# kellerberrin/KGL_Gene

Hardware: AMD Instinct MI355X
Metric: variants·genomes/sec (allele-freq sweep) (higher is better)
Workload: dtype u32

## Files before the change

### kgl_gene_amd/csrc/kgx_inbreed.hip

```cpp
#include <hip/hip_runtime.h>

#include <algorithm>
#include <cmath>
#include <cstdio>
#include <cstdlib>
#include <cstring>
#include <new>
#include <random>
#include <string>
#include <vector>

#include "kgx_kernels_inbreed.h"
#include "kgx_kernels_hall.h"
#include "kgx_kernels_loglik.h"
#include <hipcub/hipcub.hpp>
#include "kgx_internal.h"
#include "kgx_inbreed_plan.h"
#include "kgx_inbreed_buffers.h"

namespace kgx {
namespace {

int require_runtime(std::shared_ptr<Runtime>& rt) {
  rt = current_runtime();
// ... 30 lines not shown
  sw.no_eval_lut = env_int("KGX_K5_NO_EVAL_LUT", 0) != 0;
  sw.no_table_sweep = env_int("KGX_K5_NO_TABLE_SWEEP", 0) != 0;
  sw.no_swar16 = env_int("KGX_K5_NO_SWAR16", 0) != 0;
  sw.eval_gpl = env_int("KGX_K5_EVAL_GPL", 8);
  if (sw.eval_gpl != 4 && sw.eval_gpl != 8) sw.eval_gpl = 8;
  sw.blocks_per_cu = env_int("KGX_K5_BLOCKS_PER_CU", 8);
  sw.eval_resident = env_int("KGX_K5_EVAL_RESIDENT", 2);
  sw.eval_rounds = env_int("KGX_K5_EVAL_ROUNDS", 8);
  sw.sequential_min = env_int("KGX_K5_SEQUENTIAL_MIN", 1 << 16);
  sw.always_guard = env_int("KGX_K5_ALWAYS_GUARD", 0) != 0;
  sw.xcds = static_cast<uint32_t>(std::max(1, env_int("KGX_K5_XCDS", 1)));
  sw.time_small_calls = env_int("KGX_TIME_SMALL_CALLS", 0) != 0;
  sw.keep_scratch_gb = env_int("KGX_KEEP_SCRATCH_GB", -1);
  sw.no_wave = env_int("KGX_K7_NO_WAVE", 0) != 0;
  sw.wave_loci = std::min(kGenomeWaveLoci, std::max(1, env_int("KGX_K7_WAVE_LOCI", 1024)));
  sw.wave_genomes = std::max(1, env_int("KGX_K7_WAVE_GENOMES", algorithm == KGX_ALGO_HALL_ME ? 1024 : 512));
  sw.search_brent = env_str("KGX_K7_SEARCH") == "brent";
  sw.hall_passes = env_int("KGX_K7_HALL_PASSES", 0) != 0;
  sw.golden = env_int("KGX_K7_GOLDEN", 0) != 0;
  sw.estimate_start = env_int("KGX_K7_ESTIMATE_START", 0);
  sw.ll_passes = env_int("KGX_K7_LL_PASSES", 0) != 0;
  sw.ll_het_terms = env_int("KGX_K7_LL_HET_TERMS", 0) != 0;
  sw.ll_dense_per_1024 = env_int("KGX_K7_LL_DENSE_PER_1024", 0);
  sw.class_sweeps = env_int("KGX_K7_CLASS_SWEEPS", 0) != 0;
  sw.class_bytes = env_int("KGX_K7_CLASS_BYTES", 0) != 0;
  sw.order_one_lane = env_int("KGX_K7_ORDER_ONE_LANE", 0) != 0;
  sw.no_pair = env_int("KGX_K7_NO_PAIR", 0) != 0;
  sw.no_compact = env_int("KGX_K7_NO_COMPACT", 0) != 0;
  sw.compact_min_genomes = env_int("KGX_K7_COMPACT_MIN_GENOMES", 2048);
  sw.compact_min_cells = env_int("KGX_K7_COMPACT_MIN_CELLS", 1 << 26);
  sw.trace = env_int("KGX_K7_TRACE", 0) != 0;
  return sw;
}

struct ClassHits {
  unsigned long long* words = nullptr;
  uint64_t word_blocks = 0;
  bool by_bits = false;
  HallClassRows class_rows{};
};

struct EvalTarget {
  const uint32_t* gt;
  uint64_t dwords_per_row, g0, n;
  const uint32_t* index;
  double* f;
// ... 499 lines not shown
    std::fprintf(stderr, "[kgx] HallME step %d: %llu of %llu genomes moved (%llu back to the value before), largest move %.3e\n", it + 1,
                 (unsigned long long)changed, (unsigned long long)n, (unsigned long long)cycling, worst);
    trace_prev2 = trace_prev;
    trace_prev = trace_now;
  }
}

bool InbreedCall::loglik_by_moments(std::vector<uint32_t>& handed_over) {
  const uint64_t n = shape.n;
  const int objective_method = shape.objective_method;
  const bool loglik_moments = plan.loglik_candidate;
  if (objective_method == 1 && !loglik_moments)
    rc = fail(KGX_ESTATE, "kgx_inbreed_objective: this call would not run on the moments (selection size, amax, phase, memory or a switch)");
  if (!(loglik_moments && objective_method != 2 && rc == KGX_OK && gather_moments(true))) {
    if (objective_method == 1 && rc == KGX_OK)
      rc = fail(KGX_ESTATE, "kgx_inbreed_objective: a frequency without a bin, or no room for the hits' words: the passes would run");
    return false;
  }
  uint32_t* const h_totals = m.totals();
  uint32_t n_used = 0;
  try_hip(hipMemcpyAsync(&n_used, h_totals, sizeof(uint32_t), hipMemcpyDeviceToHost, st), KGX_EHIP, "D2H(used bins)");
  try_hip(hipStreamSynchronize(st), KGX_EHIP, "sync");
  unsigned long long* d_search_stats = sw.trace ? m.d_search_stats : nullptr;
  if (d_search_stats) try_hip(hipMemsetAsync(d_search_stats, 0, 8 * sizeof(unsigned long long), st), KGX_EHIP, "memset(search stats)");
  try_hip(hipEventRecord(dev.search_begin, st), KGX_EHIP, "hipEventRecord");
  hipLaunchKernelGGL(k_loglik_search, dim3(static_cast<uint32_t>(n)), dim3(kBlock), loglik_search_lds(n_used), st, m.bins, m.used(), h_totals, b.d_counts, b.d_sums,
                     m.d_smallest_het, n, plan.words_per_block, loglik_classes, b.d_start, objective_method == 1 ? 1 : 0, b.d_f, m.d_needs_passes, h_totals + 2,
                     b.d_running, d_search_stats);
  try_hip(hipGetLastError(), KGX_EHIP, "loglik search launch");
  try_hip(hipEventRecord(dev.search_end, st), KGX_EHIP, "hipEventRecord");
  search_timed = true;
  uint32_t handed = 0;
  unsigned int evaluations = 0;
  try_hip(hipMemcpyAsync(&handed, h_totals + 2, sizeof(uint32_t), hipMemcpyDeviceToHost, st), KGX_EHIP, "D2H(handed over)");
  try_hip(hipMemcpyAsync(&evaluations, b.d_running, sizeof(unsigned int), hipMemcpyDeviceToHost, st), KGX_EHIP, "D2H(evaluations)");
  try_hip(hipStreamSynchronize(st), KGX_EHIP, "sync");
  if (rc != KGX_OK) return false;
  if (d_search_stats) {
    unsigned long long stats[8] = {0};
    try_hip(hipMemcpy(stats, d_search_stats, sizeof(stats), hipMemcpyDeviceToHost), KGX_EHIP, "D2H(search stats)");
    std::fprintf(stderr, "kgx: Loglikelihood search over %llu genomes (%u bins used): %llu evaluations, %llu with cells in their band -- %llu served by kept cells, "
                         "%llu gathers kept, %llu gathers not kept, %llu dense walks; %llu cells listed, %llu blocks looked at\n",
                 (unsigned long long)n, n_used, stats[0], stats[1], stats[2], stats[3], stats[4], stats[5], stats[6], stats[7]);
  }
  dev.last_evaluations = static_cast<int>(evaluations);
  dev.last_path = KGX_PATH_LOGLIK_MOMENTS;
  if (handed) {
    std::vector<uint32_t> flags(n);
    try_hip(hipMemcpyAsync(flags.data(), m.d_needs_passes, n * sizeof(uint32_t), hipMemcpyDeviceToHost, st), KGX_EHIP, "D2H(needs passes)");
    try_hip(hipMemcpyAsync(b.d_keep, b.d_f, n * sizeof(double), hipMemcpyDeviceToDevice, st), KGX_EHIP, "copy(kept results)");
    try_hip(hipMemsetAsync(b.d_running, 0, sizeof(unsigned int), st), KGX_EHIP, "memset(running)");
    try_hip(hipStreamSynchronize(st), KGX_EHIP, "sync");
    for (uint64_t g = 0; g < n; ++g)
      if (flags[g]) {
        handed_over.push_back(static_cast<uint32_t>(g));
        if (sw.trace) std::fprintf(stderr, "kgx: Loglikelihood: genome %llu handed to the passes (reason %u)\n", (unsigned long long)(shape.g0 + g), flags[g]);
      }
    if (rc == KGX_OK) dev.last_path = KGX_PATH_LOGLIK_MOMENTS_AND_PASSES;
  }
  return true;
}

int InbreedCall::loglik_objective() {
  const uint64_t n = shape.n;
  if (shape.objective_method == 2 && rc == KGX_OK) {
    try_hip(hipMemcpyAsync(b.d_f, b.d_start, n * sizeof(double), hipMemcpyDeviceToDevice, st), KGX_EHIP, "copy(points)");
// ... 699 lines not shown
```

### kgl_gene_amd/csrc/kgx_inbreed_buffers.h

```cpp
#ifndef KGX_INBREED_BUFFERS_H
#define KGX_INBREED_BUFFERS_H

#include <type_traits>

#include "kgx_inbreed_plan.h"
#include "kgx_internal.h"
#include "kgx_kernels_loglik.h"

namespace kgx {

template <typename Fn>
void with_bool(bool value, Fn&& fn) {
  if (value) fn(std::true_type{}); else fn(std::false_type{});
}
template <int... Values, typename Fn>
void with_int(int value, Fn&& fn) {
  (void)((value == Values ? (fn(std::integral_constant<int, Values>{}), true) : false) || ...);
}

struct Carver {
  char* base = nullptr;
  ScratchPlan plan;
  template <typename T>
  T* take(size_t bytes) {
// ... 59 lines not shown
constexpr size_t kHallClassWords = 4 * (kHallBins + 1);

struct MomentsBuffers {
  uint32_t classes = 0;
  uint64_t items_per_class = 0;
  size_t padded_records = 0;
  size_t keys_bytes = 0, records_bytes = 0, sort_bytes = 0, sort_stride = 0;
  char* keys = nullptr;
  char* records = nullptr;
  HallRecord* padded = nullptr;
  uint32_t* words = nullptr;
  size_t word_count = 0;
  HallItem* items = nullptr;
  uint32_t* item_blocks = nullptr;
  double* ys = nullptr;
  int8_t* digits = nullptr;
  uint32_t* rows = nullptr;
  uint32_t* slot_of_locus = nullptr;
  char* sort = nullptr;
  double* moments = nullptr;
  double* bins = nullptr;
  uint32_t* d_needs_passes = nullptr;
  unsigned long long *d_smallest_het = nullptr, *d_search_stats = nullptr;

  uint32_t* class_words(uint32_t k) const { return words + k * kHallClassWords; }
  uint32_t* bin_used() const { return words + classes * kHallClassWords; }
  uint32_t* used() const { return bin_used() + (kHallBins + 1); }
  uint32_t* counters() const { return used() + (kHallBins + 1); }
  uint32_t* totals() const { return counters() + classes * 4; }
  HallRecord* padded_of(uint32_t k) const { return padded + static_cast<uint64_t>(k) * padded_records; }
  double* ys_of(uint32_t k) const { return ys ? ys + static_cast<uint64_t>(k) * padded_records : nullptr; }
  HallItem* items_of(uint32_t k) const { return items + static_cast<uint64_t>(k) * items_per_class; }
  uint32_t* item_blocks_of(uint32_t k) const { return item_blocks + static_cast<uint64_t>(k) * (items_per_class + 1); }
  int8_t* digits_of(uint32_t k) const { return digits + static_cast<uint64_t>(k) * padded_records * 32; }
  uint32_t* rows_of(uint32_t k) const { return rows + static_cast<uint64_t>(k) * padded_records; }
};

inline MomentsBuffers carve_moments(Carver& c, const InbreedShape& s, const InbreedPlan& p, size_t sort_bytes) {
  const uint64_t n = s.n, n_sel = s.n_sel;
  const bool planned = p.by_moments(), loglik = p.loglik_candidate;
  MomentsBuffers m;
  m.classes = planned ? p.hall_classes : 0;
  m.items_per_class = p.hall_items;
  m.padded_records = static_cast<size_t>(p.hall_blocks + 1) * kHallBlockLoci;
  m.keys_bytes = (4 * n_sel * sizeof(uint32_t) + 255) / 256 * 256;
  m.records_bytes = (n_sel * sizeof(HallRecord) + 255) / 256 * 256;
  m.keys = c.take<char>(planned ? 2 * m.keys_bytes : 0);
  m.records = c.take<char>(planned ? 2 * m.records_bytes : 0);
  m.padded = c.take<HallRecord>(m.classes * m.padded_records * sizeof(HallRecord));
  m.word_count = m.classes * kHallClassWords + 2 * (kHallBins + 1) + (m.classes + 1) * 4;
  m.words = c.take<uint32_t>(planned ? m.word_count * sizeof(uint32_t) : 0);
  m.items = c.take<HallItem>(m.classes * m.items_per_class * sizeof(HallItem));
  m.item_blocks = c.take<uint32_t>(m.classes * (m.items_per_class + 1) * sizeof(uint32_t));
  m.ys = c.take<double>(loglik ? m.classes * m.padded_records * sizeof(double) : 0);
  if (!loglik) m.ys = nullptr;
  m.digits = c.take<int8_t>(p.hall_mfma ? m.classes * m.padded_records * 32 : 0);
  m.rows = c.take<uint32_t>(p.hall_mfma ? m.classes * m.padded_records * sizeof(uint32_t) : 0);
  m.slot_of_locus = c.take<uint32_t>(p.hall_bits_planned ? m.classes * p.sel_pitch * sizeof(uint32_t) : 0);
  if (!p.hall_bits_planned) m.slot_of_locus = nullptr;
  m.sort_bytes = sort_bytes;
  m.sort_stride = (sort_bytes + 255) / 256 * 256;
  m.sort = c.take<char>(2 * m.sort_stride);
  m.moments = c.take<double>(m.items_per_class * kHallMoments * n * sizeof(double));
  m.bins = c.take<double>(planned ? static_cast<size_t>(kHallBins) * kHallMoments * n * sizeof(double) : 0);
  m.d_needs_passes = c.take<uint32_t>(loglik ? n * sizeof(uint32_t) : 0);
  m.d_smallest_het = c.take<unsigned long long>(sizeof(unsigned long long));
  m.d_search_stats = c.take<unsigned long long>(8 * sizeof(unsigned long long));
  return m;
}

}

#endif
```

### kgl_gene_amd/csrc/kgx_inbreed_plan.h

```cpp
#ifndef KGX_INBREED_PLAN_H
#define KGX_INBREED_PLAN_H

#include <cassert>
#include <cstddef>
#include <stdint.h>

#include "kgx_inbreed_constants.h"

namespace kgx {

constexpr int kAlgoRitlandLocus = 0, kAlgoSimple = 1, kAlgoHallME = 2, kAlgoLoglikelihood = 3;

struct InbreedSwitches {
  bool generic = false;
  bool no_eval_lut = false;
  bool no_table_sweep = false;
  bool no_swar16 = false;
  int eval_gpl = 8;
  int blocks_per_cu = 8;
  int eval_resident = 2;
  int eval_rounds = 8;
  int sequential_min = 1 << 16;
  bool always_guard = false;
  uint32_t xcds = 1;
  bool time_small_calls = false;
  int keep_scratch_gb = -1;
  bool no_wave = false;
  int wave_loci = 1024;
  int wave_genomes = 1024;
  bool search_brent = false;
  bool hall_passes = false;
  bool golden = false;
  int estimate_start = 0;
  bool ll_passes = false;
  bool ll_het_terms = false;
  int ll_dense_per_1024 = 0;
  bool class_sweeps = false;
  bool class_bytes = false;
  bool order_one_lane = false;
  bool no_pair = false;
  bool no_compact = false;
  int compact_min_genomes = 2048;
  int compact_min_cells = 1 << 26;
  bool trace = false;
};

struct InbreedShape {
  uint64_t n = 0;
  uint64_t g0 = 0;
  uint64_t n_sel = 0;
  uint32_t amax = 1;
  int phased = 0;
  int algorithm = kAlgoSimple;
  int objective_method = 0;
  bool has_locus_index = false;
  int compute_units = 0;
};

struct InbreedPlan {
  bool ritland = false, table_sweep = false, swar16 = false, generic_sweep = false, eval_lut = false;
  int eval_gpl = 8;
  uint32_t gx = 0, gx16 = 0;
  uint64_t n_seg = 1, per_seg = 8, eval_n_seg = 1, eval_per_seg = 8, max_seg = 1, pass_n_seg = 1;
  bool sequential_defaults = false, wave_sized = false, table_passes = false;
  int search = kSearchNelderMead, pass_search = kSearchNelderMead;
  uint64_t planes = 1;
  bool hall_candidate = false, loglik_candidate = false;
  uint32_t hall_classes = 1;
// ... 96 lines not shown
```

### kgl_gene_amd/csrc/kgx_kernels_loglik.h

```cpp
#pragma once

#include <cstdint>

#include "kgx_kernels_hall.h"

namespace kgx {

constexpr int kLoglikTmaxLog2 = 4;
constexpr double kLoglikTmax = 1.0 / (1 << kLoglikTmaxLog2);
constexpr double kLoglikBand = 1.0 / (1.0 - (1.0 / 256.0) / kLoglikTmax);
constexpr double kLoglikReach = 0.5 * kLoglikBand * (1.0 + 1.0 / 64.0);
constexpr int kLoglikMaxClasses = 15;
constexpr uint32_t kLoglikListCells = 2560;
constexpr int kLoglikWordsPerThread = 4;
constexpr double kLoglikDense = 1.0 / 4.0;
constexpr double kLogSmallProb = -23.025850929940457;
constexpr int kLoglikBinValues = 6;

struct LoglikClass {
  const double* ys;
  const uint32_t* bin_block;
  const unsigned long long* words;
};
struct LoglikClasses { LoglikClass of[kLoglikMaxClasses]; uint32_t n; uint32_t block_bins; uint32_t plain_words; uint64_t word_blocks; double dense; };

inline size_t loglik_search_lds(uint32_t n_used) {
  return static_cast<size_t>(n_used) * (kLoglikBinValues * sizeof(double) + sizeof(uint32_t)) + 8;
}

__global__ void __launch_bounds__(kBlock)
k_loglik_search(const double* __restrict__ bins, const uint32_t* __restrict__ used, const uint32_t* __restrict__ n_used_ptr,
                const unsigned long long* __restrict__ counts, const double* __restrict__ sums,
                const unsigned long long* __restrict__ smallest_het, uint64_t n_genomes, uint64_t words_per_block, LoglikClasses classes,
                const double* __restrict__ start, int mode, double* __restrict__ f_out, uint32_t* __restrict__ needs_passes,
                uint32_t* __restrict__ handed_over, unsigned int* __restrict__ max_evaluations, unsigned long long* __restrict__ stats = nullptr) {
  extern __shared__ double bin_values[];
  __shared__ double row_part[2][3][16];
  __shared__ double cell_y[kLoglikListCells];
  __shared__ uint32_t wave_total[2][kBlock / kWave];
  const uint64_t g = blockIdx.x;
  if (g >= n_genomes) return;
  const uint32_t n_used = *n_used_ptr;
  uint32_t* const bin_keys = reinterpret_cast<uint32_t*>(bin_values + static_cast<size_t>(kLoglikBinValues) * n_used);
  for (uint32_t i = threadIdx.x; i < n_used; i += kBlock) {
    const uint32_t bin = used[i];
    const double* m = bins + static_cast<uint64_t>(bin) * kHallMoments * n_genomes + g;
    double v[kLoglikBinValues] = {m[0], 0.0, 0.0, 0.0, 0.0, 0.0};
    if (bin != 0u) {
      const double r = 1.0 / hall_centre(bin);
      v[1] = m[n_genomes]; v[2] = m[2 * n_genomes] * 0.5; v[3] = m[3 * n_genomes] * (1.0 / 3.0); v[4] = m[4 * n_genomes] * 0.25;
      v[5] = r * (v[1] - r * (v[2] - r * (v[3] - r * v[4])));
    }
#pragma unroll
    for (int j = 0; j < kLoglikBinValues; ++j) bin_values[static_cast<size_t>(j) * n_used + i] = v[j];
    bin_keys[i] = bin;
  }
  __syncthreads();
  const uint32_t wave = threadIdx.x / kWave, lane = threadIdx.x % kWave;
  const uint64_t lanes = words_per_block / 8;
  int pass = 0, scans = 0;
  auto block_sum3 = [&](double& a, double& b, double& c) {
    a = row_sum16(a);
    b = row_sum16(b);
    c = row_sum16(c);
    double (*slot)[16] = row_part[pass & 1];
    if ((threadIdx.x & 15) == 0) { slot[0][threadIdx.x >> 4] = a; slot[1][threadIdx.x >> 4] = b; slot[2][threadIdx.x >> 4] = c; }
    __syncthreads();
    double out[3];
#pragma unroll
    for (int which = 0; which < 3; ++which) {
      const double* p = slot[which];
      double pair[8];
#pragma unroll
      for (int i = 0; i < 8; ++i) pair[i] = p[2 * i] + p[2 * i + 1];
      out[which] = ((pair[0] + pair[1]) + (pair[2] + pair[3])) + ((pair[4] + pair[5]) + (pair[6] + pair[7]));
    }
    a = out[0]; b = out[1]; c = out[2];
    ++pass;
  };
  auto block_scan = [&](uint32_t mine, uint32_t& total) {
    uint32_t inclusive = mine;
#pragma unroll
    for (int off = 1; off < kWave; off <<= 1) {
      const uint32_t up = __shfl_up(inclusive, off);
      if (lane >= static_cast<uint32_t>(off)) inclusive += up;
    }
    uint32_t* totals = wave_total[scans & 1];
    if (lane == kWave - 1) totals[wave] = inclusive;
    __syncthreads();
    uint32_t before = 0;
    total = 0;
#pragma unroll
    for (uint32_t w = 0; w < kBlock / kWave; ++w) {
      if (w < wave) before += totals[w];
      total += totals[w];
    }
    ++scans;
    return before + inclusive - mine;
  };
  const unsigned long long sixth = counts[g * 6 + 5], total_cells = counts[g * 6 + 4];
  const double het_big = static_cast<double>(sixth >> 32);
  const double het_tiny = static_cast<double>(total_cells - (sixth & 0xFFFFFFFFull));
  const double het_cells = static_cast<double>(counts[g * 6 + 1] + counts[g * 6 + 3]) - het_tiny;
  const double het_term = sums[g * kParts0 + 4];
  const double w_smallest = __longlong_as_double(static_cast<long long>(*smallest_het));
  uint32_t hand_over = het_big != 0.0 ? 1u : 0u;

  auto band_of = [&](double F, uint32_t& key_lo, uint32_t& key_hi) {
    const double u = 1.0 - F;
    const double disc = sqrt(__builtin_fma(F, F, 4.0 * u * 1e-10));
    const double y_floor = u > 0.0 ? (F <= 0.0 ? (disc - F) / (2.0 * u) : 2e-10 / (F + disc)) : 1e-10;
    const double y_under = y_floor * (1.0 - 1e-9), y_over = y_floor * (1.0 + 1e-9);
    key_lo = y_under < 9.5367431640625e-07 ? 1u : hall_key(y_under);
    key_hi = y_over < 9.5367431640625e-07 ? 1u : hall_key(y_over) + 1u;
    const double edge = F < 0.0 ? -F / u * kLoglikBand : 0.0;
    if (edge >= 9.5367431640625e-07) {
      const uint32_t k_edge = hall_key(edge);
      const uint32_t from = hall_centre(k_edge) < edge ? k_edge + 1u : k_edge;
      key_hi = from > key_hi ? from : key_hi;
    }
  };
  uint32_t kept_lo = 0, kept_hi = 0, kept_n = 0;

  auto objective = [&](double F, double reach_lo, double reach_hi) -> double {
    const double u = 1.0 - F;
    uint32_t key_lo, key_hi, wide_lo, wide_hi, unused;
    band_of(F, key_lo, key_hi);
    band_of(reach_hi, wide_lo, unused);
    band_of(reach_lo, unused, wide_hi);
    wide_lo = wide_lo < key_lo ? wide_lo : key_lo;
    wide_hi = wide_hi > key_hi ? wide_hi : key_hi;
    double sum = 0.0, band_cells = 0.0, wide_cells = 0.0;
    for (uint32_t i = threadIdx.x; i < n_used; i += kBlock) {
      const uint32_t key = bin_keys[i];
      const double m0 = bin_values[i];
      if (key >= key_hi) {
        const double c = hall_centre(key);
        const double A = __builtin_fma(u, c, F), t = u / A;
        const double m1 = bin_values[n_used + i], m2 = bin_values[2 * n_used + i], m3 = bin_values[3 * n_used + i], m4 = bin_values[4 * n_used + i];
        sum += __builtin_fma(m0, log(c * A), bin_values[5 * n_used + i]) + t * (m1 - t * (m2 - t * (m3 - t * m4)));
      } else if (key < key_lo) {
        sum += m0 * kLogSmallProb;
      } else {
        band_cells += m0;
      }
      if (key >= wide_lo && key < wide_hi) wide_cells += m0;
    }
    block_sum3(sum, band_cells, wide_cells);
    double value = sum;
    if (stats && threadIdx.x == 0) { atomicAdd(stats + 0, 1ull); if (band_cells > 0.0) atomicAdd(stats + 1, 1ull); }
    if (band_cells > 0.0) {
      if (key_hi > classes.block_bins || wide_hi > classes.block_bins) hand_over = 2u;
      double prod = 1.0;
      int expo = 0;
      auto exact_cell = [&](double y) {
        const double yy = y * y, d = y - yy;
        const double p = __builtin_fmin(__builtin_fmax(__builtin_fma(F, d, yy), 0.0), 1.0);
        prod *= __builtin_fmax(p, 1e-10);
      };
      auto peel = [&]() {
        expo += __builtin_amdgcn_frexp_exp(prod);
        prod = __builtin_amdgcn_frexp_mant(prod);
      };
      const bool kept_covers = kept_hi != 0u && kept_lo <= key_lo && key_hi <= kept_hi;
      const bool keep = !kept_covers && wide_cells <= static_cast<double>(kLoglikListCells);
      const uint32_t from = keep ? wide_lo : key_lo, to = keep ? wide_hi : key_hi;
      uint32_t band_blocks = 0;
      if (!kept_covers)
        for (uint32_t k = 0; k < classes.n; ++k) band_blocks += classes.of[k].bin_block[to] - classes.of[k].bin_block[from];
      const bool dense = !kept_covers && !keep && band_cells >= classes.dense * static_cast<double>(band_blocks) * kHallBlockLoci;
      auto walk_listed = [&](uint32_t n_listed) {
        for (uint32_t i0 = 0; i0 < n_listed; i0 += 8 * kBlock) {
#pragma unroll
          for (int q = 0; q < 8; ++q) {
            const uint32_t i = i0 + static_cast<uint32_t>(q) * kBlock + threadIdx.x;
            if (i < n_listed) {
              const double y = cell_y[i];
              const uint32_t key = hall_key(y);
              if (key >= key_lo && key < key_hi) exact_cell(y);
            }
          }
          peel();
        }
      };
      if (stats && threadIdx.x == 0) {
        atomicAdd(stats + (kept_covers ? 2 : dense ? 5 : keep ? 3 : 4), 1ull);
        if (!kept_covers) atomicAdd(stats + 7, static_cast<unsigned long long>(band_blocks));
      }
      if (kept_covers) {
        walk_listed(kept_n);
      } else if (dense) {
        for (uint32_t k = 0; k < classes.n && !hand_over; ++k) {
          const LoglikClass& cl = classes.of[k];
          const uint32_t b0 = cl.bin_block[key_lo], b1 = cl.bin_block[key_hi];
          for (uint32_t b = b0 + 4u * wave; b < b1; b += 16u) {
            unsigned long long word[4];
            double y[4];
#pragma unroll
            for (int q = 0; q < 4; ++q) {
              const bool in = b + q < b1;
              word[q] = in ? cl.words[classes.plain_words ? g * classes.word_blocks + (b + q) : hall_word_index(b + q, g, lanes)] : 0ull;
              y[q] = cl.ys[static_cast<uint64_t>(in ? b + q : b0) * kHallBlockLoci + lane];
            }
#pragma unroll
            for (int q = 0; q < 4; ++q)
              if ((word[q] >> (63u - lane)) & 1ull) exact_cell(y[q]);
            peel();
          }
        }
      } else {
        uint32_t listed = 0;
        kept_hi = 0u;
        uint32_t* const cell_slot = reinterpret_cast<uint32_t*>(cell_y);
        for (uint32_t k = 0; k < classes.n && !hand_over; ++k) {
          const double* const class_ys = classes.of[k].ys;
          const unsigned long long* const class_words = classes.of[k].words;
          const uint32_t b0 = classes.of[k].bin_block[from], b1 = classes.of[k].bin_block[to];
          uint32_t converted = listed;
          auto fetch_frequencies = [&]() {
            for (uint32_t i = converted + threadIdx.x; i < listed; i += kBlock) cell_y[i] = class_ys[cell_slot[2u * i]];
            converted = listed;
          };
          auto load_words = [&](uint32_t base, unsigned long long (&word)[kLoglikWordsPerThread]) {
#pragma unroll
            for (int w = 0; w < kLoglikWordsPerThread; ++w) {
              const uint32_t b = base + static_cast<uint32_t>(w) * kBlock + threadIdx.x;
              word[w] = b < b1 ? class_words[classes.plain_words ? g * classes.word_blocks + b : hall_word_index(b, g, lanes)] : 0ull;
            }
          };
          unsigned long long next_word[kLoglikWordsPerThread];
          if (b0 < b1) load_words(b0, next_word);
          for (uint32_t base = b0; base < b1; base += kBlock * kLoglikWordsPerThread) {
            unsigned long long word[kLoglikWordsPerThread];
            uint32_t mine = 0;
#pragma unroll
            for (int w = 0; w < kLoglikWordsPerThread; ++w) word[w] = next_word[w];
            if (base + kBlock * kLoglikWordsPerThread < b1) load_words(base + kBlock * kLoglikWordsPerThread, next_word);
#pragma unroll
            for (int w = 0; w < kLoglikWordsPerThread; ++w) mine += static_cast<uint32_t>(__popcll(word[w]));
            uint32_t round_total = 0;
            uint32_t at = listed + block_scan(mine, round_total);
            bool to_list = true;
            if (listed + round_total > kLoglikListCells) {
              if (keep) { hand_over = 4u; break; }
              __syncthreads();
              fetch_frequencies();
              __syncthreads();
              walk_listed(listed);
              __syncthreads();
              at -= listed;
              listed = 0;
              converted = 0;
              to_list = round_total <= kLoglikListCells;
            }
#pragma unroll
            for (int w = 0; w < kLoglikWordsPerThread; ++w) {
              const uint32_t first = (base + static_cast<uint32_t>(w) * kBlock + threadIdx.x) * kHallBlockLoci;
              unsigned long long bits = word[w];
              int walked = 0;
              while (bits != 0ull) {
                const int p = __clzll(static_cast<long long>(bits));
                bits &= ~(0x8000000000000000ull >> p);
                if (to_list) cell_slot[2u * at++] = first + static_cast<uint32_t>(p);
                else { exact_cell(class_ys[first + static_cast<uint32_t>(p)]); if ((++walked & 7) == 0) peel(); }
              }
              if (!to_list) peel();
            }
            if (to_list) listed += round_total;
          }
          __syncthreads();
          fetch_frequencies();
        }
        __syncthreads();
        if (stats && threadIdx.x == 0) atomicAdd(stats + 6, static_cast<unsigned long long>(listed));
        if (keep && !hand_over) {
          if (static_cast<double>(listed) != wide_cells) hand_over = 4u;
          kept_lo = from; kept_hi = to; kept_n = listed;
        }
        walk_listed(listed);
        if (!keep) __syncthreads();
      }
      double exact = log(prod) + static_cast<double>(expo) * 0.6931471805599453, nothing = 0.0, none = 0.0;
      block_sum3(exact, nothing, none);
      value += exact;
    }
    value += het_tiny * kLogSmallProb;
    if (het_cells > 0.0) {
      if (u * w_smallest >= 1.0000001e-10) value += het_term + het_cells * log(u);
      else if (u <= 2e-10) value += het_cells * kLogSmallProb;
      else hand_over = 3u;
    }
    return value;
  };

  if (mode == 1) {
    const double v = objective(start[g], start[g], start[g]);
    if (threadIdx.x == 0) {
      f_out[g] = hand_over ? __builtin_nan("") : v;
      needs_passes[g] = hand_over;
      if (hand_over) atomicAdd(handed_over, 1u);
    }
    return;
  }
  BrentState s = nm_start(start[g]);
  unsigned int evaluations = 0;
  for (int it = 0; it < 500 && !hand_over; ++it) {
    const double F = it == 0 ? s.x : s.u;
    const double lo = s.a < s.b ? s.a : s.b, hi = s.a < s.b ? s.b : s.a;
    const double value = objective(F, lo < F ? lo : F, hi > F ? hi : F);
    ++evaluations;
    if (hand_over) break;
    nm_advance(s, value);
    if (s.done) break;
  }
  if (threadIdx.x == 0) {
    f_out[g] = hand_over ? __builtin_nan("") : s.x;
    needs_passes[g] = hand_over;
    if (hand_over) atomicAdd(handed_over, 1u);
    atomicMax(max_evaluations, evaluations);
  }
}

__global__ void __launch_bounds__(kBlock)
k_loglik_keep(const uint32_t* __restrict__ needs_passes, const double* __restrict__ kept, uint64_t n, int planes, BrentState* __restrict__ st,
              double* __restrict__ f_next) {
  for (uint64_t g = static_cast<uint64_t>(blockIdx.x) * blockDim.x + threadIdx.x; g < n; g += static_cast<uint64_t>(gridDim.x) * blockDim.x) {
    if (needs_passes[g]) continue;
    BrentState s = st[g];
    s.done = 1;
    s.x = kept[g];
    st[g] = s;
    for (int k = 0; k < planes; ++k) f_next[k * n + g] = kept[g];
  }
}

}
```

Baseline: 24450 billion.

## Evaluate two search points per loglik pass and prune reflections with a bound

Reworks the per-genome loglikelihood search so each pass over the bins can evaluate two candidate F values at once (a paired Nelder-Mead/Brent step). The exact-cell band walk is shared across multiple class segments. Reflection steps can be rejected early when an upper bound on the band contribution already falls below the current worst value, which skips the exact cell walk. It also moves the class table to device memory, adds a tunable list-cell cap and more trace stats. The cost is more registers and LDS per block, plus a different optimizer trajectory that could change evaluation counts or hand-over behaviour.

```diff
diff --git a/kgl_gene_amd/csrc/kgx_inbreed.hip b/kgl_gene_amd/csrc/kgx_inbreed.hip
--- a/kgl_gene_amd/csrc/kgx_inbreed.hip
+++ b/kgl_gene_amd/csrc/kgx_inbreed.hip
@@ -76,6 +76,9 @@
   sw.ll_passes = env_int("KGX_K7_LL_PASSES", 0) != 0;
   sw.ll_het_terms = env_int("KGX_K7_LL_HET_TERMS", 0) != 0;
   sw.ll_dense_per_1024 = env_int("KGX_K7_LL_DENSE_PER_1024", 0);
+  static_assert(kPlanLoglikMinListCells == static_cast<int>(kLoglikMinListCells) && kPlanLoglikListCells == static_cast<int>(kLoglikListCells), "the plan's clamp is the kernel's list");
+  sw.ll_list_cells = clamp_ll_list_cells(env_int("KGX_K7_LL_LIST_CELLS", kPlanLoglikListCells));
+  sw.ll_no_bound = env_int("KGX_K7_LL_NO_BOUND", 0) != 0;
   sw.class_sweeps = env_int("KGX_K7_CLASS_SWEEPS", 0) != 0;
   sw.class_bytes = env_int("KGX_K7_CLASS_BYTES", 0) != 0;
   sw.order_one_lane = env_int("KGX_K7_ORDER_ONE_LANE", 0) != 0;
@@ -621,11 +624,14 @@
   try_hip(hipMemcpyAsync(&n_used, h_totals, sizeof(uint32_t), hipMemcpyDeviceToHost, st), KGX_EHIP, "D2H(used bins)");
   try_hip(hipStreamSynchronize(st), KGX_EHIP, "sync");
   unsigned long long* d_search_stats = sw.trace ? m.d_search_stats : nullptr;
-  if (d_search_stats) try_hip(hipMemsetAsync(d_search_stats, 0, 8 * sizeof(unsigned long long), st), KGX_EHIP, "memset(search stats)");
+  if (d_search_stats) try_hip(hipMemsetAsync(d_search_stats, 0, kLoglikStats * sizeof(unsigned long long), st), KGX_EHIP, "memset(search stats)");
+  try_hip(hipMemcpyAsync(m.d_loglik_classes, loglik_classes.of, sizeof(loglik_classes.of), hipMemcpyHostToDevice, st), KGX_EHIP, "H2D(classes)");
+  const int pair = (!sw.no_pair && objective_method != 1) ? 1 : 0;
   try_hip(hipEventRecord(dev.search_begin, st), KGX_EHIP, "hipEventRecord");
   hipLaunchKernelGGL(k_loglik_search, dim3(static_cast<uint32_t>(n)), dim3(kBlock), loglik_search_lds(n_used), st, m.bins, m.used(), h_totals, b.d_counts, b.d_sums,
-                     m.d_smallest_het, n, plan.words_per_block, loglik_classes, b.d_start, objective_method == 1 ? 1 : 0, b.d_f, m.d_needs_passes, h_totals + 2,
-                     b.d_running, d_search_stats);
+                     m.d_smallest_het, n, plan.words_per_block, m.d_loglik_classes, loglik_classes.n, loglik_classes.block_bins, loglik_classes.plain_words,
+                     loglik_classes.word_blocks, loglik_classes.dense, static_cast<uint32_t>(sw.ll_list_cells), pair, sw.ll_no_bound ? 0 : 1, b.d_start, objective_method == 1 ? 1 : 0, b.d_f,
+                     m.d_needs_passes, h_totals + 2, b.d_running, d_search_stats);
   try_hip(hipGetLastError(), KGX_EHIP, "loglik search launch");
   try_hip(hipEventRecord(dev.search_end, st), KGX_EHIP, "hipEventRecord");
   search_timed = true;
@@ -636,11 +642,12 @@
   try_hip(hipStreamSynchronize(st), KGX_EHIP, "sync");
   if (rc != KGX_OK) return false;
   if (d_search_stats) {
-    unsigned long long stats[8] = {0};
+    unsigned long long stats[kLoglikStats] = {0};
     try_hip(hipMemcpy(stats, d_search_stats, sizeof(stats), hipMemcpyDeviceToHost), KGX_EHIP, "D2H(search stats)");
     std::fprintf(stderr, "kgx: Loglikelihood search over %llu genomes (%u bins used): %llu evaluations, %llu with cells in their band -- %llu served by kept cells, "
-                         "%llu gathers kept, %llu gathers not kept, %llu dense walks; %llu cells listed, %llu blocks looked at\n",
-                 (unsigned long long)n, n_used, stats[0], stats[1], stats[2], stats[3], stats[4], stats[5], stats[6], stats[7]);
+                         "%llu gathers kept, %llu gathers not kept, %llu dense walks; %llu cells listed, %llu blocks looked at; "
+                         "%llu steps, %llu steps gathered, %llu steps served by kept cells, %llu reflections decided by their bound\n",
+                 (unsigned long long)n, n_used, stats[0], stats[1], stats[2], stats[3], stats[4], stats[5], stats[6], stats[7], stats[8], stats[9], stats[2], stats[11]);
   }
   dev.last_evaluations = static_cast<int>(evaluations);
   dev.last_path = KGX_PATH_LOGLIK_MOMENTS;
diff --git a/kgl_gene_amd/csrc/kgx_inbreed_buffers.h b/kgl_gene_amd/csrc/kgx_inbreed_buffers.h
--- a/kgl_gene_amd/csrc/kgx_inbreed_buffers.h
+++ b/kgl_gene_amd/csrc/kgx_inbreed_buffers.h
@@ -105,6 +105,7 @@
   double* bins = nullptr;
   uint32_t* d_needs_passes = nullptr;
   unsigned long long *d_smallest_het = nullptr, *d_search_stats = nullptr;
+  LoglikClass* d_loglik_classes = nullptr;
 
   uint32_t* class_words(uint32_t k) const { return words + k * kHallClassWords; }
   uint32_t* bin_used() const { return words + classes * kHallClassWords; }
@@ -148,7 +149,8 @@
   m.bins = c.take<double>(planned ? static_cast<size_t>(kHallBins) * kHallMoments * n * sizeof(double) : 0);
   m.d_needs_passes = c.take<uint32_t>(loglik ? n * sizeof(uint32_t) : 0);
   m.d_smallest_het = c.take<unsigned long long>(sizeof(unsigned long long));
-  m.d_search_stats = c.take<unsigned long long>(8 * sizeof(unsigned long long));
+  m.d_search_stats = c.take<unsigned long long>(kLoglikStats * sizeof(unsigned long long));
+  m.d_loglik_classes = c.take<LoglikClass>(loglik ? kLoglikMaxClasses * sizeof(LoglikClass) : 0);
   return m;
 }
 
diff --git a/kgl_gene_amd/csrc/kgx_inbreed_plan.h b/kgl_gene_amd/csrc/kgx_inbreed_plan.h
--- a/kgl_gene_amd/csrc/kgx_inbreed_plan.h
+++ b/kgl_gene_amd/csrc/kgx_inbreed_plan.h
@@ -35,6 +35,8 @@
   bool ll_passes = false;
   bool ll_het_terms = false;
   int ll_dense_per_1024 = 0;
+  int ll_list_cells = 2560;
+  bool ll_no_bound = false;
   bool class_sweeps = false;
   bool class_bytes = false;
   bool order_one_lane = false;
@@ -44,6 +46,11 @@
   int compact_min_cells = 1 << 26;
   bool trace = false;
 };
+
+constexpr int kPlanLoglikMinListCells = 256, kPlanLoglikListCells = 2560;
+constexpr int clamp_ll_list_cells(int asked) {
+  return asked < kPlanLoglikMinListCells ? kPlanLoglikMinListCells : asked > kPlanLoglikListCells ? kPlanLoglikListCells : asked;
+}
 
 struct InbreedShape {
   uint64_t n = 0;
diff --git a/kgl_gene_amd/csrc/kgx_kernels_loglik.h b/kgl_gene_amd/csrc/kgx_kernels_loglik.h
--- a/kgl_gene_amd/csrc/kgx_kernels_loglik.h
+++ b/kgl_gene_amd/csrc/kgx_kernels_loglik.h
@@ -1,6 +1,7 @@
 #pragma once
 
 #include <cstdint>
+#include <type_traits>
 
 #include "kgx_kernels_hall.h"
 
@@ -12,10 +13,12 @@
 constexpr double kLoglikReach = 0.5 * kLoglikBand * (1.0 + 1.0 / 64.0);
 constexpr int kLoglikMaxClasses = 15;
 constexpr uint32_t kLoglikListCells = 2560;
+constexpr uint32_t kLoglikMinListCells = 256;
 constexpr int kLoglikWordsPerThread = 4;
 constexpr double kLoglikDense = 1.0 / 4.0;
 constexpr double kLogSmallProb = -23.025850929940457;
 constexpr int kLoglikBinValues = 6;
+constexpr int kLoglikStats = 12;
 
 struct LoglikClass {
   const double* ys;
@@ -31,17 +34,32 @@
 __global__ void __launch_bounds__(kBlock)
 k_loglik_search(const double* __restrict__ bins, const uint32_t* __restrict__ used, const uint32_t* __restrict__ n_used_ptr,
                 const unsigned long long* __restrict__ counts, const double* __restrict__ sums,
-                const unsigned long long* __restrict__ smallest_het, uint64_t n_genomes, uint64_t words_per_block, LoglikClasses classes,
+                const unsigned long long* __restrict__ smallest_het, uint64_t n_genomes, uint64_t words_per_block,
+                const LoglikClass* __restrict__ class_table, uint32_t n_classes, uint32_t block_bins, uint32_t plain_words, uint64_t word_blocks,
+                double dense_share, uint32_t list_cells, int pair, int bound,
                 const double* __restrict__ start, int mode, double* __restrict__ f_out, uint32_t* __restrict__ needs_passes,
                 uint32_t* __restrict__ handed_over, unsigned int* __restrict__ max_evaluations, unsigned long long* __restrict__ stats = nullptr) {
   extern __shared__ double bin_values[];
-  __shared__ double row_part[2][3][16];
+  __shared__ double row_part[2][6][16];
   __shared__ double cell_y[kLoglikListCells];
   __shared__ uint32_t wave_total[2][kBlock / kWave];
+  __shared__ const double* class_ys[kLoglikMaxClasses];
+  __shared__ const unsigned long long* class_words[kLoglikMaxClasses];
+  __shared__ const uint32_t* class_bin_block[kLoglikMaxClasses];
+  __shared__ uint32_t seg_first[2 * kLoglikMaxClasses], seg_blocks[2 * kLoglikMaxClasses];
   const uint64_t g = blockIdx.x;
   if (g >= n_genomes) return;
   const uint32_t n_used = *n_used_ptr;
+  if (n_classes > static_cast<uint32_t>(kLoglikMaxClasses)) n_classes = kLoglikMaxClasses;
+  if (list_cells > kLoglikListCells) list_cells = kLoglikListCells;
+  const uint32_t n_segments = 2u * n_classes;
   uint32_t* const bin_keys = reinterpret_cast<uint32_t*>(bin_values + static_cast<size_t>(kLoglikBinValues) * n_used);
+  if (threadIdx.x < n_classes) {
+    const LoglikClass cl = class_table[threadIdx.x];
+    class_ys[threadIdx.x] = cl.ys;
+    class_words[threadIdx.x] = cl.words;
+    class_bin_block[threadIdx.x] = cl.bin_block;
+  }
   for (uint32_t i = threadIdx.x; i < n_used; i += kBlock) {
     const uint32_t bin = used[i];
     const double* m = bins + static_cast<uint64_t>(bin) * kHallMoments * n_genomes + g;
@@ -59,23 +77,23 @@
   const uint32_t wave = threadIdx.x / kWave, lane = threadIdx.x % kWave;
   const uint64_t lanes = words_per_block / 8;
   int pass = 0, scans = 0;
-  auto block_sum3 = [&](double& a, double& b, double& c) {
-    a = row_sum16(a);
-    b = row_sum16(b);
-    c = row_sum16(c);
+  auto block_sum = [&](auto n_tag, double (&v)[6]) {
+    constexpr int N = decltype(n_tag)::value;
     double (*slot)[16] = row_part[pass & 1];
-    if ((threadIdx.x & 15) == 0) { slot[0][threadIdx.x >> 4] = a; slot[1][threadIdx.x >> 4] = b; slot[2][threadIdx.x >> 4] = c; }
+#pragma unroll
+    for (int which = 0; which < N; ++which) {
+      v[which] = row_sum16(v[which]);
+      if ((threadIdx.x & 15) == 0) slot[which][threadIdx.x >> 4] = v[which];
+    }
     __syncthreads();
-    double out[3];
-#pragma unroll
-    for (int which = 0; which < 3; ++which) {
+#pragma unroll
+    for (int which = 0; which < N; ++which) {
       const double* p = slot[which];
-      double pair[8];
-#pragma unroll
-      for (int i = 0; i < 8; ++i) pair[i] = p[2 * i] + p[2 * i + 1];
-      out[which] = ((pair[0] + pair[1]) + (pair[2] + pair[3])) + ((pair[4] + pair[5]) + (pair[6] + pair[7]));
-    }
-    a = out[0]; b = out[1]; c = out[2];
+      double two[8];
+#pragma unroll
+      for (int i = 0; i < 8; ++i) two[i] = p[2 * i] + p[2 * i + 1];
+      v[which] = ((two[0] + two[1]) + (two[2] + two[3])) + ((two[4] + two[5]) + (two[6] + two[7]));
+    }
     ++pass;
   };
   auto block_scan = [&](uint32_t mine, uint32_t& total) {
@@ -105,6 +123,7 @@
   const double het_term = sums[g * kParts0 + 4];
   const double w_smallest = __longlong_as_double(static_cast<long long>(*smallest_het));
   uint32_t hand_over = het_big != 0.0 ? 1u : 0u;
+  uint32_t hand_over_second = 0;
 
   auto band_of = [&](double F, uint32_t& key_lo, uint32_t& key_hi) {
     const double u = 1.0 - F;
@@ -122,126 +141,239 @@
   };
   uint32_t kept_lo = 0, kept_hi = 0, kept_n = 0;
 
-  auto objective = [&](double F, double reach_lo, double reach_hi) -> double {
-    const double u = 1.0 - F;
-    uint32_t key_lo, key_hi, wide_lo, wide_hi, unused;
-    band_of(F, key_lo, key_hi);
+  auto objective = [&](auto np_tag, const double (&F)[2], double reach_lo, double reach_hi, const double (&decide_at)[2], double (&value)[2]) {
+    constexpr int NP = decltype(np_tag)::value;
+    double u[NP];
+    uint32_t key_lo[NP], key_hi[NP], wide_lo, wide_hi, unused;
+#pragma unroll
+    for (int p = 0; p < NP; ++p) {
+      u[p] = 1.0 - F[p];
+      band_of(F[p], key_lo[p], key_hi[p]);
+    }
     band_of(reach_hi, wide_lo, unused);
     band_of(reach_lo, unused, wide_hi);
-    wide_lo = wide_lo < key_lo ? wide_lo : key_lo;
-    wide_hi = wide_hi > key_hi ? wide_hi : key_hi;
-    double sum = 0.0, band_cells = 0.0, wide_cells = 0.0;
+    uint32_t first_moments = key_hi[0];
+#pragma unroll
+    for (int p = 0; p < NP; ++p) {
+      wide_lo = wide_lo < key_lo[p] ? wide_lo : key_lo[p];
+      wide_hi = wide_hi > key_hi[p] ? wide_hi : key_hi[p];
+      first_moments = first_moments < key_hi[p] ? first_moments : key_hi[p];
+    }
+    double sum[NP], band_cells[NP], wide_cells = 0.0, any_cells = 0.0;
+#pragma unroll
+    for (int p = 0; p < NP; ++p) sum[p] = band_cells[p] = 0.0;
     for (uint32_t i = threadIdx.x; i < n_used; i += kBlock) {
       const uint32_t key = bin_keys[i];
       const double m0 = bin_values[i];
-      if (key >= key_hi) {
-        const double c = hall_centre(key);
-        const double A = __builtin_fma(u, c, F), t = u / A;
-        const double m1 = bin_values[n_used + i], m2 = bin_values[2 * n_used + i], m3 = bin_values[3 * n_used + i], m4 = bin_values[4 * n_used + i];
-        sum += __builtin_fma(m0, log(c * A), bin_values[5 * n_used + i]) + t * (m1 - t * (m2 - t * (m3 - t * m4)));
-      } else if (key < key_lo) {
-        sum += m0 * kLogSmallProb;
+      double c = 0.0, m1 = 0.0, m2 = 0.0, m3 = 0.0, m4 = 0.0, series = 0.0;
+      if (key >= first_moments) {
+        c = hall_centre(key);
+        m1 = bin_values[n_used + i]; m2 = bin_values[2 * n_used + i]; m3 = bin_values[3 * n_used + i]; m4 = bin_values[4 * n_used + i];
+        series = bin_values[5 * n_used + i];
+      }
+      bool in_a_band = false;
+#pragma unroll
+      for (int p = 0; p < NP; ++p) {
+        if (key >= key_hi[p]) {
+          const double A = __builtin_fma(u[p], c, F[p]), t = u[p] / A;
+          sum[p] += __builtin_fma(m0, log(c * A), series) + t * (m1 - t * (m2 - t * (m3 - t * m4)));
+        } else if (key < key_lo[p]) {
+          sum[p] += m0 * kLogSmallProb;
+        } else {
+          band_cells[p] += m0;
+          in_a_band = true;
+        }
+      }
+      if (in_a_band) any_cells += m0;
+      if (key >= wide_lo && key < wide_hi) wide_cells += m0;
+    }
+    {
+      double v[6];
+#pragma unroll
+      for (int p = 0; p < NP; ++p) { v[p] = sum[p]; v[NP + p] = band_cells[p]; }
+      v[2 * NP] = wide_cells;
+      if constexpr (NP == 2) {
+        v[5] = any_cells;
+        block_sum(std::integral_constant<int, 6>{}, v);
+        any_cells = v[5];
       } else {
-        band_cells += m0;
-      }
-      if (key >= wide_lo && key < wide_hi) wide_cells += m0;
-    }
-    block_sum3(sum, band_cells, wide_cells);
-    double value = sum;
-    if (stats && threadIdx.x == 0) { atomicAdd(stats + 0, 1ull); if (band_cells > 0.0) atomicAdd(stats + 1, 1ull); }
-    if (band_cells > 0.0) {
-      if (key_hi > classes.block_bins || wide_hi > classes.block_bins) hand_over = 2u;
-      double prod = 1.0;
-      int expo = 0;
-      auto exact_cell = [&](double y) {
+        block_sum(std::integral_constant<int, 3>{}, v);
+        any_cells = v[1];
+      }
+#pragma unroll
+      for (int p = 0; p < NP; ++p) { value[p] = v[p]; band_cells[p] = v[NP + p]; }
+      wide_cells = v[2 * NP];
+    }
+    if (stats && threadIdx.x == 0) {
+      atomicAdd(stats + 0, static_cast<unsigned long long>(NP));
+      atomicAdd(stats + 8, 1ull);
+#pragma unroll
+      for (int p = 0; p < NP; ++p)
+        if (band_cells[p] > 0.0) atomicAdd(stats + 1, 1ull);
+    }
+    const double het_a = het_tiny * kLogSmallProb;
+    double het_b[NP], bound_term[NP];
+    bool decided[NP];
+#pragma unroll
+    for (int p = 0; p < NP; ++p) {
+      het_b[p] = 0.0;
+      if (het_cells > 0.0) {
+        if (u[p] * w_smallest >= 1.0000001e-10) het_b[p] = het_term + het_cells * log(u[p]);
+        else if (u[p] <= 2e-10) het_b[p] = het_cells * kLogSmallProb;
+        else if (p == 0) hand_over = 3u;
+        else hand_over_second = 3u;
+      }
+      decided[p] = false;
+      bound_term[p] = 0.0;
+      if (band_cells[p] > 0.0 && decide_at[p] > -__builtin_inf()) {
+        static_assert(kHallKeyMantissa >= 7, "a bin's half-width is at most 2^-8 of its centre");
+        const double y_top = hall_centre(key_hi[p] - 1u) * (1.0 + 1.0 / 256.0);
+        const double yy = y_top * y_top;
+        const double pr = __builtin_fmin(__builtin_fmax(__builtin_fma(F[p], y_top - yy, yy), 1e-10), 1.0);
+        const double most = band_cells[p] * log(pr) * (1.0 - 1e-9);
+        if (((value[p] + most) + het_a) + het_b[p] <= decide_at[p]) {
+          decided[p] = true;
+          bound_term[p] = most;
+          if constexpr (NP == 2) any_cells = band_cells[1 - p];
+          else any_cells = 0.0;
+          band_cells[p] = 0.0;
+          if (stats && threadIdx.x == 0) atomicAdd(stats + 11, 1ull);
+        }
+      }
+    }
+    if (any_cells > 0.0) {
+      uint32_t need_lo = ~0u, need_hi = 0u;
+#pragma unroll
+      for (int p = 0; p < NP; ++p) {
+        if (!(band_cells[p] > 0.0)) { key_lo[p] = key_hi[p] = 0u; continue; }
+        need_lo = need_lo < key_lo[p] ? need_lo : key_lo[p];
+        need_hi = need_hi > key_hi[p] ? need_hi : key_hi[p];
+      }
+      if (need_hi > block_bins || wide_hi > block_bins) hand_over = 2u;
+      double prod[NP];
+      int expo[NP];
+#pragma unroll
+      for (int p = 0; p < NP; ++p) { prod[p] = 1.0; expo[p] = 0; }
+      auto exact_cell = [&](double y, bool filtered) {
         const double yy = y * y, d = y - yy;
-        const double p = __builtin_fmin(__builtin_fmax(__builtin_fma(F, d, yy), 0.0), 1.0);
-        prod *= __builtin_fmax(p, 1e-10);
+        const uint32_t key = filtered ? hall_key(y) : 0u;
+#pragma unroll
+        for (int p = 0; p < NP; ++p) {
+          if (filtered && !(key >= key_lo[p] && key < key_hi[p])) continue;
+          const double pr = __builtin_fmin(__builtin_fmax(__builtin_fma(F[p], d, yy), 0.0), 1.0);
+          prod[p] *= __builtin_fmax(pr, 1e-10);
+        }
       };
       auto peel = [&]() {
-        expo += __builtin_amdgcn_frexp_exp(prod);
-        prod = __builtin_amdgcn_frexp_mant(prod);
+#pragma unroll
+        for (int p = 0; p < NP; ++p) {
+          expo[p] += __builtin_amdgcn_frexp_exp(prod[p]);
+          prod[p] = __builtin_amdgcn_frexp_mant(prod[p]);
+        }
       };
-      const bool kept_covers = kept_hi != 0u && kept_lo <= key_lo && key_hi <= kept_hi;
-      const bool keep = !kept_covers && wide_cells <= static_cast<double>(kLoglikListCells);
-      const uint32_t from = keep ? wide_lo : key_lo, to = keep ? wide_hi : key_hi;
-      uint32_t band_blocks = 0;
-      if (!kept_covers)
-        for (uint32_t k = 0; k < classes.n; ++k) band_blocks += classes.of[k].bin_block[to] - classes.of[k].bin_block[from];
-      const bool dense = !kept_covers && !keep && band_cells >= classes.dense * static_cast<double>(band_blocks) * kHallBlockLoci;
+      const bool kept_covers = kept_hi != 0u && kept_lo <= need_lo && need_hi <= kept_hi;
+      const bool keep = !kept_covers && wide_cells <= static_cast<double>(list_cells);
       auto walk_listed = [&](uint32_t n_listed) {
         for (uint32_t i0 = 0; i0 < n_listed; i0 += 8 * kBlock) {
 #pragma unroll
           for (int q = 0; q < 8; ++q) {
             const uint32_t i = i0 + static_cast<uint32_t>(q) * kBlock + threadIdx.x;
-            if (i < n_listed) {
-              const double y = cell_y[i];
-              const uint32_t key = hall_key(y);
-              if (key >= key_lo && key < key_hi) exact_cell(y);
+            if (i < n_listed) exact_cell(cell_y[i], true);
+          }
+          peel();
+        }
+      };
+      if (kept_covers) {
+        if (stats && threadIdx.x == 0) { atomicAdd(stats + 2, 1ull); atomicAdd(stats + 10, 1ull); }
+        walk_listed(kept_n);
+      } else if (!hand_over) {
+        uint32_t r_lo[2] = {keep ? wide_lo : need_lo, 0u}, r_hi[2] = {keep ? wide_hi : need_hi, 0u};
+        if constexpr (NP == 2) {
+          const int low = key_lo[0] <= key_lo[1] ? 0 : 1;
+          if (!keep && key_hi[0] != 0u && key_hi[1] != 0u && key_hi[low] < key_lo[1 - low]) {
+            r_lo[0] = key_lo[low]; r_hi[0] = key_hi[low];
+            r_lo[1] = key_lo[1 - low]; r_hi[1] = key_hi[1 - low];
+          }
+        }
+        if (threadIdx.x < n_classes) {
+          const uint32_t* const bb = class_bin_block[threadIdx.x];
+          const uint32_t a0 = bb[r_lo[0]], a1 = bb[r_hi[0]], b0 = r_hi[1] ? bb[r_lo[1]] : 0u, b1 = r_hi[1] ? bb[r_hi[1]] : 0u;
+          seg_first[2u * threadIdx.x] = a0; seg_blocks[2u * threadIdx.x] = a1 - a0;
+          seg_first[2u * threadIdx.x + 1u] = b0; seg_blocks[2u * threadIdx.x + 1u] = b1 - b0;
+        }
+        __syncthreads();
+        uint32_t band_blocks = 0;
+        for (uint32_t s = 0; s < n_segments; ++s) band_blocks += seg_blocks[s];
+        const bool dense = !keep && any_cells >= dense_share * static_cast<double>(band_blocks) * kHallBlockLoci;
+        if (stats && threadIdx.x == 0) {
+          atomicAdd(stats + (dense ? 5 : keep ? 3 : 4), 1ull);
+          atomicAdd(stats + 7, static_cast<unsigned long long>(band_blocks));
+          atomicAdd(stats + 9, 1ull);
+          atomicAdd(stats + 10, 1ull);
+        }
+        kept_hi = 0u;
+        if (dense) {
+          for (uint32_t s = 0; s < n_segments; ++s) {
+            const uint32_t b0 = seg_first[s], b1 = b0 + seg_blocks[s];
+            const double* const ys = class_ys[s >> 1];
+            const unsigned long long* const words = class_words[s >> 1];
+            for (uint32_t b = b0 + 4u * wave; b < b1; b += 16u) {
+              unsigned long long word[4];
+              double y[4];
+#pragma unroll
+              for (int q = 0; q < 4; ++q) {
+                const bool in = b + q < b1;
+                word[q] = in ? words[plain_words ? g * word_blocks + (b + q) : hall_word_index(b + q, g, lanes)] : 0ull;
+                y[q] = ys[static_cast<uint64_t>(in ? b + q : b0) * kHallBlockLoci + lane];
+              }
+#pragma unroll
+              for (int q = 0; q < 4; ++q)
+                if ((word[q] >> (63u - lane)) & 1ull) exact_cell(y[q], NP == 2);
+              peel();
             }
           }
-          peel();
-        }
-      };
-      if (stats && threadIdx.x == 0) {
-        atomicAdd(stats + (kept_covers ? 2 : dense ? 5 : keep ? 3 : 4), 1ull);
-        if (!kept_covers) atomicAdd(stats + 7, static_cast<unsigned long long>(band_blocks));
-      }
-      if (kept_covers) {
-        walk_listed(kept_n);
-      } else if (dense) {
-        for (uint32_t k = 0; k < classes.n && !hand_over; ++k) {
-          const LoglikClass& cl = classes.of[k];
-          const uint32_t b0 = cl.bin_block[key_lo], b1 = cl.bin_block[key_hi];
-          for (uint32_t b = b0 + 4u * wave; b < b1; b += 16u) {
-            unsigned long long word[4];
-            double y[4];
-#pragma unroll
-            for (int q = 0; q < 4; ++q) {
-              const bool in = b + q < b1;
-              word[q] = in ? cl.words[classes.plain_words ? g * classes.word_blocks + (b + q) : hall_word_index(b + q, g, lanes)] : 0ull;
-              y[q] = cl.ys[static_cast<uint64_t>(in ? b + q : b0) * kHallBlockLoci + lane];
+        } else {
+          uint32_t listed = 0, converted = 0;
+          uint32_t* const cell_slot = reinterpret_cast<uint32_t*>(cell_y);
+          auto fetch_frequencies = [&]() {
+            for (uint32_t i = converted + threadIdx.x; i < listed; i += kBlock) {
+              const uint32_t slot = cell_slot[2u * i], k = cell_slot[2u * i + 1u];
+              cell_y[i] = class_ys[k][slot];
             }
-#pragma unroll
-            for (int q = 0; q < 4; ++q)
-              if ((word[q] >> (63u - lane)) & 1ull) exact_cell(y[q]);
-            peel();
-          }
-        }
-      } else {
-        uint32_t listed = 0;
-        kept_hi = 0u;
-        uint32_t* const cell_slot = reinterpret_cast<uint32_t*>(cell_y);
-        for (uint32_t k = 0; k < classes.n && !hand_over; ++k) {
-          const double* const class_ys = classes.of[k].ys;
-          const unsigned long long* const class_words = classes.of[k].words;
-          const uint32_t b0 = classes.of[k].bin_block[from], b1 = classes.of[k].bin_block[to];
-          uint32_t converted = listed;
-          auto fetch_frequencies = [&]() {
-            for (uint32_t i = converted + threadIdx.x; i < listed; i += kBlock) cell_y[i] = class_ys[cell_slot[2u * i]];
             converted = listed;
           };
-          auto load_words = [&](uint32_t base, unsigned long long (&word)[kLoglikWordsPerThread]) {
+          uint32_t cursor_s = 0, cursor_from = 0, cursor_to = seg_blocks[0];
+          auto load_words = [&](uint32_t base, unsigned long long (&word)[kLoglikWordsPerThread], uint32_t (&first)[kLoglikWordsPerThread],
+                                uint32_t (&of_class)[kLoglikWordsPerThread]) {
 #pragma unroll
             for (int w = 0; w < kLoglikWordsPerThread; ++w) {
-              const uint32_t b = base + static_cast<uint32_t>(w) * kBlock + threadIdx.x;
-              word[w] = b < b1 ? class_words[classes.plain_words ? g * classes.word_blocks + b : hall_word_index(b, g, lanes)] : 0ull;
+              const uint32_t v = base + static_cast<uint32_t>(w) * kBlock + threadIdx.x;
+              word[w] = 0ull; first[w] = 0u; of_class[w] = 0u;
+              if (v < band_blocks) {
+                while (v >= cursor_to) { ++cursor_s; cursor_from = cursor_to; cursor_to += seg_blocks[cursor_s]; }
+                const uint32_t b = seg_first[cursor_s] + (v - cursor_from);
+                of_class[w] = cursor_s >> 1;
+                first[w] = b * kHallBlockLoci;
+                word[w] = class_words[cursor_s >> 1][plain_words ? g * word_blocks + b : hall_word_index(b, g, lanes)];
+              }
             }
           };
           unsigned long long next_word[kLoglikWordsPerThread];
-          if (b0 < b1) load_words(b0, next_word);
-          for (uint32_t base = b0; base < b1; base += kBlock * kLoglikWordsPerThread) {
+          uint32_t next_first[kLoglikWordsPerThread], next_class[kLoglikWordsPerThread];
+          if (band_blocks != 0u) load_words(0u, next_word, next_first, next_class);
+          for (uint32_t base = 0; base < band_blocks; base += kBlock * kLoglikWordsPerThread) {
             unsigned long long word[kLoglikWordsPerThread];
+            uint32_t first[kLoglikWordsPerThread], of_class[kLoglikWordsPerThread];
             uint32_t mine = 0;
 #pragma unroll
-            for (int w = 0; w < kLoglikWordsPerThread; ++w) word[w] = next_word[w];
-            if (base + kBlock * kLoglikWordsPerThread < b1) load_words(base + kBlock * kLoglikWordsPerThread, next_word);
+            for (int w = 0; w < kLoglikWordsPerThread; ++w) { word[w] = next_word[w]; first[w] = next_first[w]; of_class[w] = next_class[w]; }
+            if (base + kBlock * kLoglikWordsPerThread < band_blocks) load_words(base + kBlock * kLoglikWordsPerThread, next_word, next_first, next_class);
 #pragma unroll
             for (int w = 0; w < kLoglikWordsPerThread; ++w) mine += static_cast<uint32_t>(__popcll(word[w]));
             uint32_t round_total = 0;
             uint32_t at = listed + block_scan(mine, round_total);
             bool to_list = true;
-            if (listed + round_total > kLoglikListCells) {
+            if (listed + round_total > list_cells) {
               if (keep) { hand_over = 4u; break; }
               __syncthreads();
               fetch_frequencies();
@@ -251,18 +383,18 @@
               at -= listed;
               listed = 0;
               converted = 0;
-              to_list = round_total <= kLoglikListCells;
+              to_list = round_total <= list_cells;
             }
 #pragma unroll
             for (int w = 0; w < kLoglikWordsPerThread; ++w) {
-              const uint32_t first = (base + static_cast<uint32_t>(w) * kBlock + threadIdx.x) * kHallBlockLoci;
               unsigned long long bits = word[w];
+              const double* const ys = to_list ? nullptr : class_ys[of_class[w]];
               int walked = 0;
               while (bits != 0ull) {
                 const int p = __clzll(static_cast<long long>(bits));
                 bits &= ~(0x8000000000000000ull >> p);
-                if (to_list) cell_slot[2u * at++] = first + static_cast<uint32_t>(p);
-                else { exact_cell(class_ys[first + static_cast<uint32_t>(p)]); if ((++walked & 7) == 0) peel(); }
+                if (to_list) { cell_slot[2u * at] = first[w] + static_cast<uint32_t>(p); cell_slot[2u * at + 1u] = of_class[w]; ++at; }
+                else { exact_cell(ys[first[w] + static_cast<uint32_t>(p)], NP == 2); if ((++walked & 7) == 0) peel(); }
               }
               if (!to_list) peel();
             }
@@ -270,54 +402,78 @@
           }
           __syncthreads();
           fetch_frequencies();
-        }
-        __syncthreads();
-        if (stats && threadIdx.x == 0) atomicAdd(stats + 6, static_cast<unsigned long long>(listed));
-        if (keep && !hand_over) {
-          if (static_cast<double>(listed) != wide_cells) hand_over = 4u;
-          kept_lo = from; kept_hi = to; kept_n = listed;
-        }
-        walk_listed(listed);
-        if (!keep) __syncthreads();
-      }
-      double exact = log(prod) + static_cast<double>(expo) * 0.6931471805599453, nothing = 0.0, none = 0.0;
-      block_sum3(exact, nothing, none);
-      value += exact;
-    }
-    value += het_tiny * kLogSmallProb;
-    if (het_cells > 0.0) {
-      if (u * w_smallest >= 1.0000001e-10) value += het_term + het_cells * log(u);
-      else if (u <= 2e-10) value += het_cells * kLogSmallProb;
-      else hand_over = 3u;
-    }
-    return value;
+          __syncthreads();
+          if (stats && threadIdx.x == 0) atomicAdd(stats + 6, static_cast<unsigned long long>(listed));
+          if (keep && !hand_over) {
+            if (static_cast<double>(listed) != wide_cells) hand_over = 4u;
+            kept_lo = r_lo[0]; kept_hi = r_hi[0]; kept_n = listed;
+          }
+          walk_listed(listed);
+          if (!keep) __syncthreads();
+        }
+      }
+      {
+        double v[6];
+#pragma unroll
+        for (int p = 0; p < NP; ++p) v[p] = log(prod[p]) + static_cast<double>(expo[p]) * 0.6931471805599453;
+        if constexpr (NP == 2) {
+          block_sum(std::integral_constant<int, 2>{}, v);
+        } else {
+          v[1] = v[2] = 0.0;
+          block_sum(std::integral_constant<int, 3>{}, v);
+        }
+#pragma unroll
+        for (int p = 0; p < NP; ++p) value[p] += v[p];
+      }
+    }
+#pragma unroll
+    for (int p = 0; p < NP; ++p) {
+      if (decided[p]) value[p] += bound_term[p];
+      value[p] = (value[p] + het_a) + het_b[p];
+    }
   };
 
-  if (mode == 1) {
-    const double v = objective(start[g], start[g], start[g]);
-    if (threadIdx.x == 0) {
-      f_out[g] = hand_over ? __builtin_nan("") : v;
-      needs_passes[g] = hand_over;
-      if (hand_over) atomicAdd(handed_over, 1u);
-    }
-    return;
-  }
-  BrentState s = nm_start(start[g]);
+  BrentState s = pair && mode == 0 ? nm2_start(start[g]) : nm_start(start[g]);
   unsigned int evaluations = 0;
   for (int it = 0; it < 500 && !hand_over; ++it) {
-    const double F = it == 0 ? s.x : s.u;
     const double lo = s.a < s.b ? s.a : s.b, hi = s.a < s.b ? s.b : s.a;
-    const double value = objective(F, lo < F ? lo : F, hi > F ? hi : F);
+    double F[2] = {mode == 1 ? start[g] : s.u, s.d}, value[2];
+    const bool two = pair && mode == 0 && s.u != s.d;
+    const bool reflection = bound && mode == 0 && (pair ? two && s.widened == kNm2Reflect : s.widened == kNmReflect);
+    const double decide_at[2] = {reflection ? s.fw : -__builtin_inf(), -__builtin_inf()};
+    if (two) {
+      const double lo2 = F[0] < F[1] ? F[0] : F[1], hi2 = F[0] < F[1] ? F[1] : F[0];
+      objective(std::integral_constant<int, 2>{}, F, lo < lo2 ? lo : lo2, hi > hi2 ? hi : hi2, decide_at, value);
+    } else if (mode == 1) {
+      objective(std::integral_constant<int, 1>{}, F, F[0], F[0], decide_at, value);
+    } else {
+      objective(std::integral_constant<int, 1>{}, F, lo < F[0] ? lo : F[0], hi > F[0] ? hi : F[0], decide_at, value);
+    }
+    if (mode == 1) {
+      if (threadIdx.x == 0) {
+        f_out[g] = hand_over ? __builtin_nan("") : value[0];
+        needs_passes[g] = hand_over;
+        if (hand_over) atomicAdd(handed_over, 1u);
+      }
+      return;
+    }
     ++evaluations;
-    if (hand_over) break;
-    nm_advance(s, value);
+    if (pair) {
+      if (two && hand_over_second && !hand_over && (s.widened == kNm2Start || !(value[0] > s.fw))) hand_over = hand_over_second;
+      hand_over_second = 0;
+      if (hand_over) break;
+      nm2_advance(s, value[0], two ? value[1] : value[0]);
+    } else {
+      if (hand_over) break;
+      nm_advance(s, value[0]);
+    }
     if (s.done) break;
   }
   if (threadIdx.x == 0) {
     f_out[g] = hand_over ? __builtin_nan("") : s.x;
     needs_passes[g] = hand_over;
     if (hand_over) atomicAdd(handed_over, 1u);
-    atomicMax(max_evaluations, evaluations);
+    atomicMax(max_evaluations, pair && !hand_over ? static_cast<unsigned int>(s.e) : evaluations);
   }
 }
 
```

Result: no change. 24410 billion (-0.2%).
